# fema-ffrd/gpras

Measured on AMD Instinct MI355X. Metric: gp_fits_per_sec, higher is better.
Workload: dtype f64; 1 GPU; BASELINE configs[1] as the many-independent-cells workload: exact GP N=4096 d=8 RBF, fit F1 = kernel build + blocked fp64-MFMA Cholesky + alpha + LML, per cell; cells = y columns of one training set with per-cell hyperparameters (the reference's per-mode models); n_train=4096, d=8, kernel=RBF, collective=none (one process), launcher=single process

## Files before the change

gpras_amd/csrc/potrf.h:

```cpp
#pragma once
#include <cstdlib>
#include <utility>
#include <vector>

#include "chain64.h"
#include "gemm_f64.h"
#include "gprx_common.h"

namespace gprx {

#ifdef GPRX_PANEL_ACC
__device__ unsigned long long g_panel_acc[8];
#define PACC_DECL unsigned long long pacc_prev_ = 0;
#define PACC(i)                                                                                                       \
  {                                                                                                                   \
    if ((i) == 5) __builtin_amdgcn_s_waitcnt(0);                                                                      \
    const unsigned long long t_ = __builtin_amdgcn_s_memtime();                                                       \
    if (threadIdx.x == 0 && blockIdx.x == 0 && blockIdx.y == 0 && gridDim.x > 2) {                                    \
      if ((i) > 0) atomicAdd(&g_panel_acc[i], t_ - pacc_prev_);                                                       \
      else atomicAdd(&g_panel_acc[0], 1ull);                                                                          \
    }                                                                                                                 \
    pacc_prev_ = t_;                                                                                                  \
  }
#else
#define PACC_DECL
#define PACC(i)
#endif
#ifdef GPRX_PANEL_STAMPS
__device__ unsigned long long g_panel_stamps[64];
#define PSTAMP(i)                                                                                                     \
  if (threadIdx.x == 0) {                                                                                             \
    if (blockIdx.x == 0) g_panel_stamps[i] = __builtin_amdgcn_s_memtime();                                            \
    if (blockIdx.x == gridDim.x / 2 && (i) < 6) g_panel_stamps[32 + (i)] = __builtin_amdgcn_s_memtime();               \
    if (blockIdx.x == gridDim.x - 2 && (i) < 6) g_panel_stamps[48 + (i)] = __builtin_amdgcn_s_memtime();               \
  }
#else
#define PSTAMP(i)
#endif

constexpr int RT = 2;
constexpr int PANEL_WG_ROWS = 64 * RT;
constexpr int PANEL_OWN_ROWS = PANEL_WG_ROWS - NB;

struct PanelCtx {
  double* sIn;
  double* sX;
  double* out;
  double* inv_diag;
  double* rinv_out;
  int ident;
  int tid, wave, g, r;
  int zero_above;
  int bad;
};

template <int P>
__device__ __forceinline__ void panel_step(d4 (&acc)[RT][4], PanelCtx& c) {
  constexpr int WROWS = 16 * RT;
  constexpr int PWG_ROWS = PANEL_WG_ROWS;
  constexpr int C0 = 8 * P;
  constexpr int KT = C0 / 16;
  constexpr int HALF = P & 1;
  if constexpr (P == 1) { PSTAMP(10) }
  if ((c.r >> 3) == HALF) {
#pragma unroll
    for (int rt = 0; rt < RT; ++rt)
#pragma unroll
      for (int q = 0; q < 4; ++q) c.sIn[(WROWS * c.wave + 16 * rt + c.g + 4 * q) * PSUB + (c.r & 7)] = acc[rt][KT][q];
  }
  __syncthreads();
  if constexpr (P == 1) { PSTAMP(11) }
  double l[8][8], rinv[8];
#pragma unroll
  for (int j = 0; j < 8; ++j)
#pragma unroll
    for (int k = 0; k <= j; ++k) l[j][k] = c.sIn[(C0 + j) * PSUB + k];
#pragma unroll
  for (int j = 0; j < 8; ++j) {
    double s = l[j][j];
#pragma unroll
    for (int m = 0; m < j; ++m) s = __builtin_fma(-l[j][m], l[j][m], s);
    if (!(s > 0.0)) {
      if (c.bad == 0) c.bad = C0 + j + 1;
      s = 1.0;
    }
    const double ri = rsqrt_f64(s);
    rinv[j] = ri;
    l[j][j] = s * ri;
#pragma unroll
    for (int i = j + 1; i < 8; ++i) {
      double t = l[i][j];
#pragma unroll
      for (int m = 0; m < j; ++m) t = __builtin_fma(-l[i][m], l[j][m], t);
      l[i][j] = t * ri;
    }
  }
  if (c.rinv_out && c.tid == 0) {
#pragma unroll
    for (int j = 0; j < 8; ++j) c.rinv_out[C0 + j] = rinv[j];
  }
  if constexpr (P == 1) { PSTAMP(12) }
  if (c.tid < PWG_ROWS) {
    double x[8];
#pragma unroll
    for (int k = 0; k < 8; ++k) {
      double t = c.sIn[c.tid * PSUB + k];
#pragma unroll
      for (int m = 0; m < k; ++m) t = __builtin_fma(-x[m], l[k][m], t);
      x[k] = (C0 + k > c.zero_above) ? 0.0 : t * rinv[k];
    }
    if constexpr (P == 1) { PSTAMP(16) }
#pragma unroll
    for (int k = 0; k < 8; ++k) c.sX[c.tid * PSUB + k] = x[k];
    if constexpr (P == 1) { PSTAMP(17) }
    if (c.out) {
#pragma unroll
      for (int k = 0; k < 8; k += 2) *reinterpret_cast<d2*>(c.out + C0 + k) = d2{x[k], x[k + 1]};
    }
    if (c.ident >= 0) {
#pragma unroll
      for (int k = 0; k < 8; ++k) c.inv_diag[(C0 + k) * NB + c.ident] = x[k];
    }
  }
  if constexpr (P == 1) { PSTAMP(13) }
  __syncthreads();
  if constexpr (P == 1) { PSTAMP(14) }
  if constexpr (C0 + 8 < NB) {
    constexpr int KT0 = (C0 + 8) / 16;
    double fa[RT][2], fb[4][2];
#pragma unroll
    for (int rt = 0; rt < RT; ++rt)
#pragma unroll
      for (int ks = 0; ks < 2; ++ks) fa[rt][ks] = -c.sX[(WROWS * c.wave + 16 * rt + c.r) * PSUB + 4 * ks + c.g];
#pragma unroll
    for (int kt = KT0; kt < 4; ++kt) {
      const int kk = kt * 16 + c.r;
#pragma unroll
      for (int ks = 0; ks < 2; ++ks) fb[kt][ks] = (kk >= C0 + 8) ? c.sX[kk * PSUB + 4 * ks + c.g] : 0.0;
    }
#pragma unroll
    for (int kt = KT0; kt < 4; ++kt)
#pragma unroll
      for (int rt = 0; rt < RT; ++rt) {
        acc[rt][kt] = __builtin_amdgcn_mfma_f64_16x16x4f64(fa[rt][0], fb[kt][0], acc[rt][kt], 0, 0, 0);
        acc[rt][kt] = __builtin_amdgcn_mfma_f64_16x16x4f64(fa[rt][1], fb[kt][1], acc[rt][kt], 0, 0, 0);
      }
  }
  if ((c.r >> 3) == HALF) {
#pragma unroll
    for (int rt = 0; rt < RT; ++rt)
#pragma unroll
      for (int q = 0; q < 4; ++q) acc[rt][KT][q] = c.sX[(WROWS * c.wave + 16 * rt + c.g + 4 * q) * PSUB + (c.r & 7)];
  }
  if constexpr (P == 1) { PSTAMP(15) }
}

__device__ __forceinline__ void flush_staged_block(const double* __restrict__ prev_stage, double* __restrict__ prev_dst, int64_t lda,
                                                   int prev_pw, int tid) {
  if (!prev_stage) return;
  const int chunks = prev_pw / 2;
  for (int e = tid; e < prev_pw * chunks; e += 256) {
    const int row = e / chunks, cc = e % chunks;
    *reinterpret_cast<d2*>(prev_dst + (int64_t)row * lda + 2 * cc) = *reinterpret_cast<const d2*>(prev_stage + row * prev_pw + 2 * cc);
  }
}

__global__ __launch_bounds__(256) void copy_block_kernel(const double* __restrict__ stage, double* __restrict__ dst, int64_t lda, int pw,
                                                         int64_t cs) {
  flush_staged_block(stage + (int64_t)blockIdx.x * cs, dst + (int64_t)blockIdx.x * cs, lda, pw, threadIdx.x);
}

template <bool FUSE_K64>
__global__ __launch_bounds__(256, 2) void potrf_panel_kernel(double* __restrict__ A, int64_t lda, int rows_below, int nchunks,
                                                          double* __restrict__ inv_diag, int* __restrict__ info, int col0,
                                                          double* __restrict__ stage_out, const double* __restrict__ prev_stage,
                                                          double* __restrict__ prev_dst, int prev_pw, int64_t cs, int info_stride,
                                                          double* __restrict__ yv) {
  constexpr int PWG_ROWS = PANEL_WG_ROWS;
  constexpr int PANEL_ROWS = PANEL_OWN_ROWS;
  constexpr int WROWS = 16 * RT;
#ifndef GPRX_PANEL_NO_SETPRIO
  __builtin_amdgcn_s_setprio(3);
#endif
  {
    const int64_t off = (int64_t)blockIdx.y * cs;
    A += off;
    inv_diag += off;
    stage_out += off;
    if (prev_stage) prev_stage += off;
    if (prev_dst) prev_dst += off;
    info += (int64_t)blockIdx.y * info_stride;
  }
  __shared__ __attribute__((aligned(16))) double sIn[PWG_ROWS * PSUB];
  __shared__ __attribute__((aligned(16))) double sX[PWG_ROWS * PSUB];
  PanelCtx c;
  c.sIn = sIn;
  c.sX = sX;
  c.inv_diag = inv_diag;
  c.tid = threadIdx.x;
  const int lane = c.tid & 63;
  c.wave = c.tid >> 6;
  c.g = lane >> 4;
  c.r = lane & 15;
  c.zero_above = c.tid < NB ? c.tid : (1 << 30);
  c.bad = 0;
  const bool last = (int)blockIdx.x == nchunks;
  c.rinv_out = last ? stage_out + NB * NB : nullptr;
  if (last) flush_staged_block(prev_stage, prev_dst, lda, prev_pw, c.tid);
  c.out = nullptr;
  c.ident = -1;
  if (c.tid < NB) {
    if (last) c.out = stage_out + c.tid * NB;
  } else if (c.tid < PWG_ROWS) {
    if (last && c.tid < 2 * NB) c.ident = c.tid - NB;
  }
  PSTAMP(0)
  PACC_DECL
  PACC(0)

  d4 acc[RT][4];
  {
    const double* rowp[RT][4];
    bool valid[RT][4];
#pragma unroll
    for (int rt = 0; rt < RT; ++rt)
#pragma unroll
      for (int q = 0; q < 4; ++q) {
        const int wrow = WROWS * c.wave + 16 * rt + c.g + 4 * q;
        const int idx = (int)blockIdx.x * PANEL_ROWS + (wrow - NB);
        const bool diag = wrow < NB;
        const bool ok = diag || (!last && idx < rows_below);
        const int64_t mrow = diag ? wrow : (ok ? NB + idx : 0);
        rowp[rt][q] = A + mrow * lda + c.r;
        valid[rt][q] = ok;
      }
    d4 upd[FUSE_K64 ? RT : 1][4];
    if constexpr (FUSE_K64) {
#pragma unroll
      for (int rt = 0; rt < RT; ++rt)
#pragma unroll
        for (int kt = 0; kt < 4; ++kt) upd[rt][kt] = d4{0.0, 0.0, 0.0, 0.0};
      const double* arow[RT];
#pragma unroll
      for (int rt = 0; rt < RT; ++rt) {
        const int wrow = WROWS * c.wave + 16 * rt + c.r;
        const int idx = (int)blockIdx.x * PANEL_ROWS + (wrow - NB);
        const bool diag = wrow < NB;
        const bool ok = diag || (!last && idx < rows_below);
        arow[rt] = A + (diag ? wrow : (ok ? NB + idx : 0)) * lda - NB + 4 * c.g;
      }
      const double* brow = A + (int64_t)c.r * lda - NB + 4 * c.g;
#pragma unroll
      for (int k0 = 0; k0 < NB; k0 += 16) {
        double fa[RT][4], fb[4][4];
#pragma unroll
        for (int rt = 0; rt < RT; ++rt) {
          const d2 lo = *reinterpret_cast<const d2*>(arow[rt] + k0), hi = *reinterpret_cast<const d2*>(arow[rt] + k0 + 2);
          fa[rt][0] = lo.x; fa[rt][1] = lo.y; fa[rt][2] = hi.x; fa[rt][3] = hi.y;
        }
#pragma unroll
        for (int kt = 0; kt < 4; ++kt) {
          const double* bp = brow + (int64_t)(16 * kt) * lda + k0;
          const d2 lo = *reinterpret_cast<const d2*>(bp), hi = *reinterpret_cast<const d2*>(bp + 2);
          fb[kt][0] = lo.x; fb[kt][1] = lo.y; fb[kt][2] = hi.x; fb[kt][3] = hi.y;
        }
#pragma unroll
        for (int j = 0; j < 4; ++j)
#pragma unroll
          for (int rt = 0; rt < RT; ++rt)
#pragma unroll
            for (int kt = 0; kt < 4; ++kt) upd[rt][kt] = __builtin_amdgcn_mfma_f64_16x16x4f64(fa[rt][j], fb[kt][j], upd[rt][kt], 0, 0, 0);
      }
    }
#pragma unroll
    for (int rt = 0; rt < RT; ++rt)
#pragma unroll
      for (int q = 0; q < 4; ++q)
#pragma unroll
        for (int kt = 0; kt < 4; ++kt) acc[rt][kt][q] = rowp[rt][q][kt * 16];
    if constexpr (FUSE_K64) {
#pragma unroll
      for (int rt = 0; rt < RT; ++rt)
#pragma unroll
        for (int kt = 0; kt < 4; ++kt)
#pragma unroll
          for (int q = 0; q < 4; ++q) {
            const double v = -1.0 * upd[rt][kt][q];
            acc[rt][kt][q] = __builtin_fma(1.0, acc[rt][kt][q], v);
          }
    }
#pragma unroll
    for (int rt = 0; rt < RT; ++rt)
#pragma unroll
      for (int q = 0; q < 4; ++q) {
        const int wrow = WROWS * c.wave + 16 * rt + c.g + 4 * q;
#pragma unroll
        for (int kt = 0; kt < 4; ++kt) {
          const int col = kt * 16 + c.r;
          double v = valid[rt][q] ? acc[rt][kt][q] : 0.0;
          if (wrow < NB) {
            v = (col > wrow) ? 0.0 : v;
          } else if (last) {
            v = (col == wrow - NB) ? 1.0 : 0.0;
          }
          acc[rt][kt][q] = v;
        }
      }
  }
  PSTAMP(1)
  PACC(1)

  panel_step<0>(acc, c);
  PSTAMP(2)
  PACC(2)
  panel_step<1>(acc, c);
  panel_step<2>(acc, c);
  panel_step<3>(acc, c);
  PSTAMP(3)
  PACC(3)
  panel_step<4>(acc, c);
  panel_step<5>(acc, c);
  panel_step<6>(acc, c);
  panel_step<7>(acc, c);
  PSTAMP(4)
  PACC(4)
  if (!last) {
#pragma unroll
    for (int rt = 0; rt < RT; ++rt)
#pragma unroll
      for (int q = 0; q < 4; ++q) {
        const int wrow = WROWS * c.wave + 16 * rt + c.g + 4 * q;
        const int idx = (int)blockIdx.x * PANEL_ROWS + (wrow - NB);
        if (wrow >= NB && idx < rows_below) {
          double* dst = A + (int64_t)(NB + idx) * lda + c.r;
#pragma unroll
          for (int kt = 0; kt < 4; ++kt) dst[kt * 16] = acc[rt][kt][q];
        }
      }
  }
  if (last && c.tid == 0 && c.bad != 0) atomicCAS(info, 0, col0 + c.bad);
  if (yv != nullptr && last) {
    yv += (int64_t)blockIdx.y * cs;
    asm volatile("s_waitcnt vmcnt(0)" ::: "memory");
    __syncthreads();
    double* sv = sIn;
    double* sred = sIn + NB;
    static_assert(PWG_ROWS * PSUB >= NB + 256, "the sub-panel buffer holds y_j and the partial sums");
    if (c.tid < NB) sv[c.tid] = yv[c.tid];
    __syncthreads();
    const int a = c.tid & 63, qq = c.tid >> 6;
    const double* row = inv_diag + a * NB + 16 * qq;
    double sum = 0.0;
#pragma unroll
    for (int i = 0; i < 16; ++i) sum = __builtin_fma(row[i], sv[16 * qq + i], sum);
    sred[c.tid] = sum;
    __syncthreads();
    if (c.tid < NB) yv[c.tid] = ((sred[c.tid] + sred[64 + c.tid]) + sred[128 + c.tid]) + sred[192 + c.tid];
  }
  PSTAMP(5)
  PACC(5)
}

constexpr int ROWS_WG = 64 * RT;
__device__ __forceinline__ void wave_sync_lds() {
  __builtin_amdgcn_fence(__ATOMIC_RELEASE, "wavefront");
  __builtin_amdgcn_wave_barrier();
  __builtin_amdgcn_fence(__ATOMIC_ACQUIRE, "wavefront");
}
template <int P>
__device__ __forceinline__ void rows_step(d4 (&acc)[RT][4], double* __restrict__ sIn, double* __restrict__ sX, int tid, int wave, int g, int r,
                                          const double* __restrict__ gstage) {
  constexpr int C0 = 8 * P;
  constexpr int KT = C0 / 16;
  constexpr int HALF = P & 1;
  constexpr int WROWS = 16 * RT;
  if ((r >> 3) == HALF) {
#pragma unroll
    for (int rt = 0; rt < RT; ++rt)
#pragma unroll
      for (int q = 0; q < 4; ++q) sIn[(WROWS * wave + 16 * rt + g + 4 * q) * PSUB + (r & 7)] = acc[rt][KT][q];
  }
  wave_sync_lds();
  const int srow = WROWS * wave + (tid & 63);
  if ((tid & 63) < WROWS) {
    double x[8];
#pragma unroll
    for (int k = 0; k < 8; ++k) {
      double t = sIn[srow * PSUB + k];
#pragma unroll
      for (int m = 0; m < k; ++m) t = __builtin_fma(-x[m], gstage[(C0 + k) * NB + C0 + m], t);
      x[k] = t * gstage[NB * NB + C0 + k];
    }
#pragma unroll
    for (int k = 0; k < 8; ++k) sX[srow * PSUB + k] = x[k];
  }
  wave_sync_lds();
  if constexpr (C0 + 8 < NB) {
    constexpr int KT0 = (C0 + 8) / 16;
    double fa[RT][2], fb[4][2];
#pragma unroll
    for (int rt = 0; rt < RT; ++rt)
#pragma unroll
      for (int ks = 0; ks < 2; ++ks) fa[rt][ks] = -sX[(WROWS * wave + 16 * rt + r) * PSUB + 4 * ks + g];
#pragma unroll
    for (int kt = KT0; kt < 4; ++kt) {
      const int kk = kt * 16 + r;
#pragma unroll
      for (int ks = 0; ks < 2; ++ks) fb[kt][ks] = (kk >= C0 + 8) ? gstage[kk * NB + C0 + 4 * ks + g] : 0.0;
    }
#pragma unroll
    for (int kt = KT0; kt < 4; ++kt)
#pragma unroll
      for (int rt = 0; rt < RT; ++rt) {
        acc[rt][kt] = __builtin_amdgcn_mfma_f64_16x16x4f64(fa[rt][0], fb[kt][0], acc[rt][kt], 0, 0, 0);
        acc[rt][kt] = __builtin_amdgcn_mfma_f64_16x16x4f64(fa[rt][1], fb[kt][1], acc[rt][kt], 0, 0, 0);
      }
  }
  if ((r >> 3) == HALF) {
#pragma unroll
    for (int rt = 0; rt < RT; ++rt)
#pragma unroll
      for (int q = 0; q < 4; ++q) acc[rt][KT][q] = sX[(WROWS * wave + 16 * rt + g + 4 * q) * PSUB + (r & 7)];
  }
}

template <bool FUSE_K64, bool YVEC>
__global__ __launch_bounds__(256, FUSE_K64 ? 2 : 4) void potrf_rows_kernel(double* __restrict__ A21, int64_t lda, int rows_below,
                                                                           const double* __restrict__ stage, int64_t cs, double* __restrict__ yv) {
  constexpr int WG_ROWS = ROWS_WG, WROWS = 16 * RT;
  __shared__ __attribute__((aligned(16))) double sIn[WG_ROWS * PSUB];
  __shared__ __attribute__((aligned(16))) double sX[WG_ROWS * PSUB];
  A21 += (int64_t)blockIdx.y * cs;
  stage += (int64_t)blockIdx.y * cs;
  const int tid = threadIdx.x, lane = tid & 63, wave = tid >> 6, g = lane >> 4, r = lane & 15;
  const int row0 = blockIdx.x * WG_ROWS;
  d4 acc[RT][4];
  {
    const double* rowp[RT][4];
    bool valid[RT][4];
#pragma unroll
    for (int rt = 0; rt < RT; ++rt)
#pragma unroll
      for (int q = 0; q < 4; ++q) {
        const int idx = row0 + WROWS * wave + 16 * rt + g + 4 * q;
        valid[rt][q] = idx < rows_below;
        rowp[rt][q] = A21 + (int64_t)(valid[rt][q] ? idx : 0) * lda + r;
      }
    d4 upd[FUSE_K64 ? RT : 1][4];
    if constexpr (FUSE_K64) {
#pragma unroll
      for (int rt = 0; rt < RT; ++rt)
#pragma unroll
        for (int kt = 0; kt < 4; ++kt) upd[rt][kt] = d4{0.0, 0.0, 0.0, 0.0};
      const double* arow[RT];
#pragma unroll
      for (int rt = 0; rt < RT; ++rt) {
        const int idx = row0 + WROWS * wave + 16 * rt + r;
        arow[rt] = A21 + (int64_t)(idx < rows_below ? idx : 0) * lda - NB + 4 * g;
      }
      const double* brow = A21 - (int64_t)NB * lda + (int64_t)r * lda - NB + 4 * g;
#pragma unroll
      for (int k0 = 0; k0 < NB; k0 += 16) {
        double fa[RT][4], fb[4][4];
#pragma unroll
        for (int rt = 0; rt < RT; ++rt) {
          const d2 lo = *reinterpret_cast<const d2*>(arow[rt] + k0), hi = *reinterpret_cast<const d2*>(arow[rt] + k0 + 2);
          fa[rt][0] = lo.x; fa[rt][1] = lo.y; fa[rt][2] = hi.x; fa[rt][3] = hi.y;
        }
#pragma unroll
        for (int kt = 0; kt < 4; ++kt) {
          const double* bp = brow + (int64_t)(16 * kt) * lda + k0;
          const d2 lo = *reinterpret_cast<const d2*>(bp), hi = *reinterpret_cast<const d2*>(bp + 2);
          fb[kt][0] = lo.x; fb[kt][1] = lo.y; fb[kt][2] = hi.x; fb[kt][3] = hi.y;
        }
#pragma unroll
        for (int j = 0; j < 4; ++j)
#pragma unroll
          for (int rt = 0; rt < RT; ++rt)
#pragma unroll
            for (int kt = 0; kt < 4; ++kt) upd[rt][kt] = __builtin_amdgcn_mfma_f64_16x16x4f64(fa[rt][j], fb[kt][j], upd[rt][kt], 0, 0, 0);
      }
    }
#pragma unroll
    for (int rt = 0; rt < RT; ++rt)
#pragma unroll
      for (int q = 0; q < 4; ++q)
#pragma unroll
        for (int kt = 0; kt < 4; ++kt) acc[rt][kt][q] = rowp[rt][q][kt * 16];
    if constexpr (FUSE_K64) {
#pragma unroll
      for (int rt = 0; rt < RT; ++rt)
#pragma unroll
        for (int kt = 0; kt < 4; ++kt)
#pragma unroll
          for (int q = 0; q < 4; ++q) {
            const double v = -1.0 * upd[rt][kt][q];
            acc[rt][kt][q] = __builtin_fma(1.0, acc[rt][kt][q], v);
          }
    }
#pragma unroll
    for (int rt = 0; rt < RT; ++rt)
#pragma unroll
      for (int q = 0; q < 4; ++q)
#pragma unroll
        for (int kt = 0; kt < 4; ++kt) acc[rt][kt][q] = valid[rt][q] ? acc[rt][kt][q] : 0.0;
  }
  rows_step<0>(acc, sIn, sX, tid, wave, g, r, stage);
  rows_step<1>(acc, sIn, sX, tid, wave, g, r, stage);
  rows_step<2>(acc, sIn, sX, tid, wave, g, r, stage);
  rows_step<3>(acc, sIn, sX, tid, wave, g, r, stage);
  rows_step<4>(acc, sIn, sX, tid, wave, g, r, stage);
  rows_step<5>(acc, sIn, sX, tid, wave, g, r, stage);
  double ybj[YVEC ? 4 : 1], yold[YVEC ? RT : 1][4];
  if constexpr (YVEC) {
    yv += (int64_t)blockIdx.y * cs;
#pragma unroll
    for (int kt = 0; kt < 4; ++kt) ybj[kt] = yv[16 * kt + r];
#pragma unroll
    for (int rt = 0; rt < RT; ++rt)
#pragma unroll
      for (int q = 0; q < 4; ++q) {
        const int idx = row0 + WROWS * wave + 16 * rt + g + 4 * q;
        yold[rt][q] = yv[NB + (idx < rows_below ? idx : 0)];
      }
  }
  rows_step<6>(acc, sIn, sX, tid, wave, g, r, stage);
  rows_step<7>(acc, sIn, sX, tid, wave, g, r, stage);
#pragma unroll
  for (int rt = 0; rt < RT; ++rt)
#pragma unroll
    for (int q = 0; q < 4; ++q) {
      const int idx = row0 + WROWS * wave + 16 * rt + g + 4 * q;
      if (idx < rows_below) {
        double* dst = A21 + (int64_t)idx * lda + r;
#pragma unroll
        for (int kt = 0; kt < 4; ++kt) dst[kt * 16] = acc[rt][kt][q];
      }
    }
  if constexpr (YVEC) {
#pragma unroll
    for (int rt = 0; rt < RT; ++rt)
#pragma unroll
      for (int q = 0; q < 4; ++q) {
        double sum = acc[rt][0][q] * ybj[0];
#pragma unroll
        for (int kt = 1; kt < 4; ++kt) sum = __builtin_fma(acc[rt][kt][q], ybj[kt], sum);
#pragma unroll
        for (int m = 1; m < 16; m <<= 1) sum += __shfl_xor(sum, m, 64);
        const int idx = row0 + WROWS * wave + 16 * rt + g + 4 * q;
        if (r == 0 && idx < rows_below) yv[NB + idx] = yold[rt][q] - sum;
      }
  }
}

constexpr int STAGE_LD = 129;

struct PotrfProfile {
  std::vector<hipEvent_t> pool;
  size_t used = 0;
  std::vector<std::pair<size_t, double>> gemm_marks;
  std::vector<std::pair<size_t, double>> strip_marks;
  std::vector<size_t> panel_marks;
  hipEvent_t next() {
    if (used == pool.size()) {
      hipEvent_t e;
      hipEventCreate(&e);
      pool.push_back(e);
    }
    return pool[used++];
  }
  void reset() {
    used = 0;
    gemm_marks.clear();
    strip_marks.clear();
    panel_marks.clear();
  }
  ~PotrfProfile() {
    for (auto e : pool) hipEventDestroy(e);
  }
};

struct PotrfTuning {
  int outer_block = 0;
  int update_tile = 0;
  int no_lookahead = 0;
  int split_panel = 0;
  int poison_workspace = 0;
  int cell_kernel = 0;
  int rhs_vector = 0;
  int dag = 0;
};
inline PotrfTuning& potrf_tuning() {
  static PotrfTuning t = [] {
    PotrfTuning v;
    if (const char* e = getenv("GPRX_OUTER_BLOCK")) v.outer_block = atoi(e);
    if (const char* e = getenv("GPRX_UPDATE_TILE")) v.update_tile = atoi(e);
    if (const char* e = getenv("GPRX_SPLIT_PANEL")) v.split_panel = atoi(e);
    if (const char* e = getenv("GPRX_DAG")) v.dag = atoi(e);
    if (const char* e = getenv("GPRX_RHS_VECTOR")) v.rhs_vector = atoi(e);
    if (const char* e = getenv("GPRX_CELL_KERNEL")) v.cell_kernel = atoi(e);
    return v;
  }();
  return t;
}

struct PotrfStreams {
  hipStream_t aux = nullptr;
  hipEvent_t block_done = nullptr, tail_done = nullptr;
  hipError_t init() {
    hipError_t e = hipStreamCreateWithFlags(&aux, hipStreamNonBlocking);
    if (e != hipSuccess) return e;
    if ((e = hipEventCreateWithFlags(&block_done, hipEventDisableTiming)) != hipSuccess) return e;
    return hipEventCreateWithFlags(&tail_done, hipEventDisableTiming);
  }
  void destroy() {
    if (aux) hipStreamDestroy(aux);
    if (block_done) hipEventDestroy(block_done);
    if (tail_done) hipEventDestroy(tail_done);
    aux = nullptr;
    block_done = tail_done = nullptr;
  }
};

inline bool potrf_split_panel(const PotrfTuning& tune, int batch) { return tune.split_panel ? tune.split_panel > 0 : batch >= 24; }

inline bool potrf_rhs_vector_ok(const PotrfTuning& tune, int batch) { return tune.rhs_vector >= 0 && batch > 1 && potrf_split_panel(tune, batch); }

inline hipError_t potrf_lower(hipStream_t st, double* A, int64_t lda, int np, int extra, double* inv_diag, int* info,
                              double* diag_stage, PotrfProfile* prof = nullptr, PotrfStreams* ps = nullptr, int batch = 1, int64_t cs = 0,
                              int info_stride = 0, const PotrfTuning* tune_in = nullptr, int col_base = 0, double* yvec = nullptr) {
  const double* prev_stage = nullptr;
  double* prev_dst = nullptr;
  auto mark_gemm = [&](hipStream_t s, int ncols_lower, int rows_rect, int ncols, int k, bool strip = false) {
    if (!prof) return;
    const double elems = 0.5 * (double)ncols_lower * (ncols_lower + 1) + (double)rows_rect * ncols;
    (strip ? prof->strip_marks : prof->gemm_marks).push_back({prof->used, 2.0 * k * elems * batch});
    hipEventRecord(prof->next(), s);
  };
  auto mark_end = [&](hipStream_t s) {
    if (prof) hipEventRecord(prof->next(), s);
  };
  const int total_rows = np + extra;
  const PotrfTuning& tune = tune_in ? *tune_in : potrf_tuning();
  if (tune.no_lookahead) ps = nullptr;
  const int ob = tune.outer_block ? tune.outer_block : (np > 4096 ? 512 : 1024);
  const int bulk_tile = tune.update_tile ? tune.update_tile : 64;
  bool tail_pending = false;
  hipError_t err = hipSuccess;
  const bool split_panel = potrf_split_panel(tune, batch);
  if (yvec && !split_panel) return hipErrorInvalidValue;
  auto panel = [&](int c, bool fuse = false) {
    const int rows_below = total_rows - c - NB;
    double* Acc = A + (int64_t)c * lda + c;
    if (prof) {
      prof->panel_marks.push_back(prof->used);
      hipEventRecord(prof->next(), st);
    }
    double* stage_out = diag_stage + (int64_t)c * STAGE_LD;
    double* invd = inv_diag + (int64_t)(c / NB) * NB * NB;
    double* yv = yvec ? yvec + c : nullptr;
    const int own_rows = split_panel ? 0 : rows_below;
    const int nchunks = (own_rows + PANEL_OWN_ROWS - 1) / PANEL_OWN_ROWS;
    const auto diag = fuse ? potrf_panel_kernel<true> : potrf_panel_kernel<false>;
    hipLaunchKernelGGL(diag, dim3(nchunks + 1, batch), dim3(256), 0, st, Acc, lda,
                       own_rows, nchunks, invd, info, col_base + c, stage_out, prev_stage, prev_dst, NB, cs, info_stride, yv);
    if (split_panel && rows_below > 0) {
      const auto rows = fuse ? (yv ? potrf_rows_kernel<true, true> : potrf_rows_kernel<true, false>)
                             : (yv ? potrf_rows_kernel<false, true> : potrf_rows_kernel<false, false>);
      hipLaunchKernelGGL(rows, dim3((rows_below + ROWS_WG - 1) / ROWS_WG, batch), dim3(256), 0, st, Acc + (int64_t)NB * lda, lda, rows_below,
                         (const double*)stage_out, cs, yv);
    }
    prev_stage = stage_out;
    prev_dst = Acc;
    if (prof) hipEventRecord(prof->next(), st);
  };
  auto update = [&](int c0, int k, int c1, int n, int tile) {
    const int rows = total_rows - c1;
    const double* L21 = A + (int64_t)c1 * lda + c0;
    double* A22 = A + (int64_t)c1 * lda + c1;
    mark_gemm(st, n, rows - n, n, k, k <= 128);
    hipError_t e = launch_gemm(st, 0, 1, rows, n, k, -1.0, L21, lda, L21, lda, 1.0, A22, lda, GEMM_C_LOWER, k == NB ? 64 : tile, batch, cs, cs, cs);
    mark_end(st);
    if (e != hipSuccess && err == hipSuccess) err = e;
  };
  auto factor_range = [&](auto&& self, int c0, int w) -> void {
    if (w <= NB) {
      panel(c0);
      return;
    }
    const int h = ((w / NB + 1) / 2) * NB;
    self(self, c0, h);
    if (h == NB && w - h == NB) {
      panel(c0 + h, true);
      return;
    }
    update(c0, h, c0 + h, w - h, 64);
    self(self, c0 + h, w - h);
  };
  for (int C = 0; C < np; C += ob) {
    const int w = (np - C < ob) ? np - C : ob;
    factor_range(factor_range, C, w);
    if (err != hipSuccess) return err;
    const int R = C + w;
    if (R >= np) break;
    const int wn = (np - R < ob) ? np - R : ob;
    if (ps && tail_pending) hipStreamWaitEvent(st, ps->tail_done, 0);
    update(C, w, R, wn, batch > 1 ? bulk_tile : 64);
    if (err != hipSuccess) return err;
    if (ps) hipEventRecord(ps->block_done, st);
    const int R2 = R + wn;
    if (R2 < np) {
      hipStream_t ts = ps ? ps->aux : st;
      if (ps) hipStreamWaitEvent(ts, ps->block_done, 0);
      const int rows = total_rows - R2, cols = np - R2;
      const double* Lrow = A + (int64_t)R2 * lda + C;
      mark_gemm(ts, cols, rows - cols, cols, w);
      hipError_t e = launch_gemm(ts, 0, 1, rows, cols, w, -1.0, Lrow, lda, Lrow, lda, 1.0, A + (int64_t)R2 * lda + R2, lda, GEMM_C_LOWER,
                                   bulk_tile, batch, cs, cs, cs);
      mark_end(ts);
      if (e != hipSuccess) return e;
      if (ps) {
        hipEventRecord(ps->tail_done, ts);
        tail_pending = true;
      }
    }
  }
  if (prev_stage) hipLaunchKernelGGL(copy_block_kernel, dim3(batch), dim3(256), 0, st, prev_stage, prev_dst, lda, NB, cs);
  if (ps && tail_pending) hipStreamWaitEvent(st, ps->tail_done, 0);
  return hipGetLastError();
}

}
```

Measured before the change: 2192 fits/s.

## Stage panel diagonal and trailing fragments into LDS via async DMA in rows kernel

The rows kernel now copies the diagonal 8x8 sub-blocks, inverse diagonal, y head and the panel fragments needed by each rows_step into LDS with global-to-LDS DMA at kernel start. In the fused-K64 path the copy is issued after the GEMM update so it overlaps with that work. The triangular solve and MFMA B-operand reads then come from LDS instead of repeated scattered global loads. Register pressure is cut by holding one yold value per lane instead of an RT x 4 array, and launch bounds rise to 3 workgroups for the fused variant. The costs are more shared memory per workgroup and an extra block-wide barrier.

New measurement: 2205 fits/s, median of 6. About the same (+0.6%).

```diff
diff --git a/gpras_amd/csrc/potrf.h b/gpras_amd/csrc/potrf.h
--- a/gpras_amd/csrc/potrf.h
+++ b/gpras_amd/csrc/potrf.h
@@ -367,9 +367,29 @@
   __builtin_amdgcn_wave_barrier();
   __builtin_amdgcn_fence(__ATOMIC_ACQUIRE, "wavefront");
 }
+constexpr int ROWS_SUB_DOUBLES = 8 * 64 + 4 * NB;
+constexpr int rows_frag_base(int P) {
+  int n = 0;
+  for (int p = 0; p < P; ++p) n += 4 - (8 * p + 8) / 16;
+  return n;
+}
+constexpr int ROWS_FRAG_DOUBLES = rows_frag_base(7) * 128;
+static_assert(rows_frag_base(7) == 16, "four DMA instructions per wave of a four-wave workgroup");
+constexpr int rows_frag_src(int idx) {
+  int P = 0;
+  while (rows_frag_base(P + 1) <= idx) ++P;
+  return (16 * ((8 * P + 8) / 16 + idx - rows_frag_base(P))) * NB + 8 * P;
+}
+static_assert(rows_frag_src(0) == 0 && rows_frag_src(4) == 16 * NB + 8 && rows_frag_src(15) == 48 * NB + 48, "pieces in step order, kt ascending");
+template <int J>
+__device__ __forceinline__ void rows_frag_dma(const double* __restrict__ gstage, double* __restrict__ sF, int wave, unsigned piece_lane) {
+  constexpr int S0 = rows_frag_src(4 * J), S1 = rows_frag_src(4 * J + 1), S2 = rows_frag_src(4 * J + 2), S3 = rows_frag_src(4 * J + 3);
+  const int src = (wave & 2) ? ((wave & 1) ? S3 : S2) : ((wave & 1) ? S1 : S0);
+  glds16(gstage + src + piece_lane, sF + 128 * (4 * J + wave));
+}
 template <int P>
 __device__ __forceinline__ void rows_step(d4 (&acc)[RT][4], double* __restrict__ sIn, double* __restrict__ sX, int tid, int wave, int g, int r,
-                                          const double* __restrict__ gstage) {
+                                          const double* __restrict__ sD, const double* __restrict__ sF) {
   constexpr int C0 = 8 * P;
   constexpr int KT = C0 / 16;
   constexpr int HALF = P & 1;
@@ -388,15 +408,15 @@
     for (int k = 0; k < 8; ++k) {
       double t = sIn[srow * PSUB + k];
 #pragma unroll
-      for (int m = 0; m < k; ++m) t = __builtin_fma(-x[m], gstage[(C0 + k) * NB + C0 + m], t);
-      x[k] = t * gstage[NB * NB + C0 + k];
+      for (int m = 0; m < k; ++m) t = __builtin_fma(-x[m], sD[64 * P + 8 * k + m], t);
+      x[k] = t * sD[8 * 64 + C0 + k];
     }
 #pragma unroll
     for (int k = 0; k < 8; ++k) sX[srow * PSUB + k] = x[k];
   }
   wave_sync_lds();
   if constexpr (C0 + 8 < NB) {
-    constexpr int KT0 = (C0 + 8) / 16;
+    constexpr int KT0 = (C0 + 8) / 16, PIECE0 = rows_frag_base(P);
     double fa[RT][2], fb[4][2];
 #pragma unroll
     for (int rt = 0; rt < RT; ++rt)
@@ -406,7 +426,8 @@
     for (int kt = KT0; kt < 4; ++kt) {
       const int kk = kt * 16 + r;
 #pragma unroll
-      for (int ks = 0; ks < 2; ++ks) fb[kt][ks] = (kk >= C0 + 8) ? gstage[kk * NB + C0 + 4 * ks + g] : 0.0;
+      for (int ks = 0; ks < 2; ++ks)
+        fb[kt][ks] = (kk >= C0 + 8) ? sF[(PIECE0 + kt - KT0) * 128 + 64 * ks + 32 * (g >> 1) + 2 * r + (g & 1)] : 0.0;
     }
 #pragma unroll
     for (int kt = KT0; kt < 4; ++kt)
@@ -425,17 +446,71 @@
 }
 
 template <bool FUSE_K64, bool YVEC>
-__global__ __launch_bounds__(256, FUSE_K64 ? 2 : 4) void potrf_rows_kernel(double* __restrict__ A21, int64_t lda, int rows_below,
+__global__ __launch_bounds__(256, FUSE_K64 ? 3 : 4) void potrf_rows_kernel(double* __restrict__ A21, int64_t lda, int rows_below,
                                                                            const double* __restrict__ stage, int64_t cs, double* __restrict__ yv) {
   constexpr int WG_ROWS = ROWS_WG, WROWS = 16 * RT;
-  __shared__ __attribute__((aligned(16))) double sIn[WG_ROWS * PSUB];
-  __shared__ __attribute__((aligned(16))) double sX[WG_ROWS * PSUB];
+  __shared__ __attribute__((aligned(16))) double smem[2 * WG_ROWS * PSUB + ROWS_SUB_DOUBLES + ROWS_FRAG_DOUBLES];
+  static_assert(sizeof(smem) <= 40 * 1024, "four workgroups per CU");
+  double* const sIn = smem;
+  double* const sX = sIn + WG_ROWS * PSUB;
+  double* const sD = sX + WG_ROWS * PSUB;
+  double* const sF = sD + ROWS_SUB_DOUBLES;
   A21 += (int64_t)blockIdx.y * cs;
   stage += (int64_t)blockIdx.y * cs;
-  const int tid = threadIdx.x, lane = tid & 63, wave = tid >> 6, g = lane >> 4, r = lane & 15;
+  if constexpr (YVEC) yv += (int64_t)blockIdx.y * cs;
+  const int tid = threadIdx.x, lane = tid & 63, g = lane >> 4, r = lane & 15;
+  const int wave = __builtin_amdgcn_readfirstlane(tid >> 6);
   const int row0 = blockIdx.x * WG_ROWS;
+  auto stage_dma = [&] {
+    const unsigned h8 = 8 * (lane >> 5);
+    glds16(stage + 16 * wave * (NB + 1) + ((h8 + ((lane >> 2) & 7)) * NB + h8 + 2 * (lane & 3)), sD + 128 * wave);
+    if (wave == 0) glds16(stage + NB * NB + 2u * (lane & 31), sD + 8 * 64);
+    if (YVEC && wave == 1) glds16(yv + 2u * (lane & 31), sD + 8 * 64 + 2 * NB);
+    const unsigned piece_lane = (lane & 15) * NB + 2 * (lane >> 4);
+    rows_frag_dma<0>(stage, sF, wave, piece_lane);
+    rows_frag_dma<1>(stage, sF, wave, piece_lane);
+    rows_frag_dma<2>(stage, sF, wave, piece_lane);
+    rows_frag_dma<3>(stage, sF, wave, piece_lane);
+  };
+  if constexpr (!FUSE_K64) stage_dma();
   d4 acc[RT][4];
   {
+    d4 upd[FUSE_K64 ? RT : 1][4];
+    if constexpr (FUSE_K64) {
+#pragma unroll
+      for (int rt = 0; rt < RT; ++rt)
+#pragma unroll
+        for (int kt = 0; kt < 4; ++kt) upd[rt][kt] = d4{0.0, 0.0, 0.0, 0.0};
+      const double* arow[RT];
+#pragma unroll
+      for (int rt = 0; rt < RT; ++rt) {
+        const int idx = row0 + WROWS * wave + 16 * rt + r;
+        arow[rt] = A21 + (int64_t)(idx < rows_below ? idx : 0) * lda - NB + 4 * g;
+      }
+      const double* bblock = A21 - (int64_t)NB * lda - NB;
+      const unsigned blane = (unsigned)r * (unsigned)lda + 4 * g;
+#pragma unroll
+      for (int k0 = 0; k0 < NB; k0 += 16) {
+        double fa[RT][4], fb[4][4];
+#pragma unroll
+        for (int rt = 0; rt < RT; ++rt) {
+          const d2 lo = *reinterpret_cast<const d2*>(arow[rt] + k0), hi = *reinterpret_cast<const d2*>(arow[rt] + k0 + 2);
+          fa[rt][0] = lo.x; fa[rt][1] = lo.y; fa[rt][2] = hi.x; fa[rt][3] = hi.y;
+        }
+#pragma unroll
+        for (int kt = 0; kt < 4; ++kt) {
+          const double* bp = bblock + (int64_t)(16 * kt) * lda + k0 + blane;
+          const d2 lo = *reinterpret_cast<const d2*>(bp), hi = *reinterpret_cast<const d2*>(bp + 2);
+          fb[kt][0] = lo.x; fb[kt][1] = lo.y; fb[kt][2] = hi.x; fb[kt][3] = hi.y;
+        }
+#pragma unroll
+        for (int j = 0; j < 4; ++j)
+#pragma unroll
+          for (int rt = 0; rt < RT; ++rt)
+#pragma unroll
+            for (int kt = 0; kt < 4; ++kt) upd[rt][kt] = __builtin_amdgcn_mfma_f64_16x16x4f64(fa[rt][j], fb[kt][j], upd[rt][kt], 0, 0, 0);
+      }
+    }
     const double* rowp[RT][4];
     bool valid[RT][4];
 #pragma unroll
@@ -446,41 +521,6 @@
         valid[rt][q] = idx < rows_below;
         rowp[rt][q] = A21 + (int64_t)(valid[rt][q] ? idx : 0) * lda + r;
       }
-    d4 upd[FUSE_K64 ? RT : 1][4];
-    if constexpr (FUSE_K64) {
-#pragma unroll
-      for (int rt = 0; rt < RT; ++rt)
-#pragma unroll
-        for (int kt = 0; kt < 4; ++kt) upd[rt][kt] = d4{0.0, 0.0, 0.0, 0.0};
-      const double* arow[RT];
-#pragma unroll
-      for (int rt = 0; rt < RT; ++rt) {
-        const int idx = row0 + WROWS * wave + 16 * rt + r;
-        arow[rt] = A21 + (int64_t)(idx < rows_below ? idx : 0) * lda - NB + 4 * g;
-      }
-      const double* brow = A21 - (int64_t)NB * lda + (int64_t)r * lda - NB + 4 * g;
-#pragma unroll
-      for (int k0 = 0; k0 < NB; k0 += 16) {
-        double fa[RT][4], fb[4][4];
-#pragma unroll
-        for (int rt = 0; rt < RT; ++rt) {
-          const d2 lo = *reinterpret_cast<const d2*>(arow[rt] + k0), hi = *reinterpret_cast<const d2*>(arow[rt] + k0 + 2);
-          fa[rt][0] = lo.x; fa[rt][1] = lo.y; fa[rt][2] = hi.x; fa[rt][3] = hi.y;
-        }
-#pragma unroll
-        for (int kt = 0; kt < 4; ++kt) {
-          const double* bp = brow + (int64_t)(16 * kt) * lda + k0;
-          const d2 lo = *reinterpret_cast<const d2*>(bp), hi = *reinterpret_cast<const d2*>(bp + 2);
-          fb[kt][0] = lo.x; fb[kt][1] = lo.y; fb[kt][2] = hi.x; fb[kt][3] = hi.y;
-        }
-#pragma unroll
-        for (int j = 0; j < 4; ++j)
-#pragma unroll
-          for (int rt = 0; rt < RT; ++rt)
-#pragma unroll
-            for (int kt = 0; kt < 4; ++kt) upd[rt][kt] = __builtin_amdgcn_mfma_f64_16x16x4f64(fa[rt][j], fb[kt][j], upd[rt][kt], 0, 0, 0);
-      }
-    }
 #pragma unroll
     for (int rt = 0; rt < RT; ++rt)
 #pragma unroll
@@ -488,6 +528,7 @@
 #pragma unroll
         for (int kt = 0; kt < 4; ++kt) acc[rt][kt][q] = rowp[rt][q][kt * 16];
     if constexpr (FUSE_K64) {
+      stage_dma();
 #pragma unroll
       for (int rt = 0; rt < RT; ++rt)
 #pragma unroll
@@ -505,27 +546,22 @@
 #pragma unroll
         for (int kt = 0; kt < 4; ++kt) acc[rt][kt][q] = valid[rt][q] ? acc[rt][kt][q] : 0.0;
   }
-  rows_step<0>(acc, sIn, sX, tid, wave, g, r, stage);
-  rows_step<1>(acc, sIn, sX, tid, wave, g, r, stage);
-  rows_step<2>(acc, sIn, sX, tid, wave, g, r, stage);
-  rows_step<3>(acc, sIn, sX, tid, wave, g, r, stage);
-  rows_step<4>(acc, sIn, sX, tid, wave, g, r, stage);
-  rows_step<5>(acc, sIn, sX, tid, wave, g, r, stage);
-  double ybj[YVEC ? 4 : 1], yold[YVEC ? RT : 1][4];
+  __syncthreads();
+  rows_step<0>(acc, sIn, sX, tid, wave, g, r, sD, sF);
+  rows_step<1>(acc, sIn, sX, tid, wave, g, r, sD, sF);
+  rows_step<2>(acc, sIn, sX, tid, wave, g, r, sD, sF);
+  rows_step<3>(acc, sIn, sX, tid, wave, g, r, sD, sF);
+  rows_step<4>(acc, sIn, sX, tid, wave, g, r, sD, sF);
+  rows_step<5>(acc, sIn, sX, tid, wave, g, r, sD, sF);
+  static_assert(4 * RT <= 16, "a lane group of 16 holds an entry of y per row");
+  double yold = 0.0;
   if constexpr (YVEC) {
-    yv += (int64_t)blockIdx.y * cs;
-#pragma unroll
-    for (int kt = 0; kt < 4; ++kt) ybj[kt] = yv[16 * kt + r];
-#pragma unroll
-    for (int rt = 0; rt < RT; ++rt)
-#pragma unroll
-      for (int q = 0; q < 4; ++q) {
-        const int idx = row0 + WROWS * wave + 16 * rt + g + 4 * q;
-        yold[rt][q] = yv[NB + (idx < rows_below ? idx : 0)];
-      }
-  }
-  rows_step<6>(acc, sIn, sX, tid, wave, g, r, stage);
-  rows_step<7>(acc, sIn, sX, tid, wave, g, r, stage);
+    const int idx = row0 + WROWS * wave + 16 * ((r >> 2) % RT) + g + 4 * (r & 3);
+    yold = yv[NB + (idx < rows_below ? idx : 0)];
+  }
+  rows_step<6>(acc, sIn, sX, tid, wave, g, r, sD, sF);
+  rows_step<7>(acc, sIn, sX, tid, wave, g, r, sD, sF);
+  if constexpr (YVEC) asm volatile("" : "+v"(yold));
 #pragma unroll
   for (int rt = 0; rt < RT; ++rt)
 #pragma unroll
@@ -538,6 +574,9 @@
       }
     }
   if constexpr (YVEC) {
+    double ybj[4];
+#pragma unroll
+    for (int kt = 0; kt < 4; ++kt) ybj[kt] = sD[8 * 64 + 2 * NB + 16 * kt + r];
 #pragma unroll
     for (int rt = 0; rt < RT; ++rt)
 #pragma unroll
@@ -548,7 +587,7 @@
 #pragma unroll
         for (int m = 1; m < 16; m <<= 1) sum += __shfl_xor(sum, m, 64);
         const int idx = row0 + WROWS * wave + 16 * rt + g + 4 * q;
-        if (r == 0 && idx < rows_below) yv[NB + idx] = yold[rt][q] - sum;
+        if (r == 4 * rt + q && idx < rows_below) yv[NB + idx] = yold - sum;
       }
   }
 }
```
